# blachlylab/fade

Hardware: AMD Instinct MI355X
Metric: annotate reads/sec at 1/2/4/8 MI355X; rs/am tag bit-exact vs ref (higher is better)
Workload: dtype int16; 1 GPU; C2: 10000000 x 150 bp PE reads per GPU per step in 10 distinct batches, -w 100, --min-length 5, p_softclip 0.10; slots_in_flight=2, records_left_out=none

## Files before the change

fade_amd/csrc/fadehip.hip:

```cpp
#include "fadehip_kernels.hpp"
#include "bgzf_deflate.hpp"
#include "bgzf_inflate.hpp"
#include "bam_device.hpp"
#include "sw_stats.hpp"
#include <rccl/rccl.h>
#include <algorithm>
#include <chrono>
#include <condition_variable>
#include <cstdarg>
#include <cstdio>
#include <cstdlib>
#include <cstring>
#include <ctime>
#include <map>
#include <mutex>
#include <new>
#include <string>
#include <thread>
#include <unordered_map>
#include <vector>

using namespace fadehip;

namespace {
// ... 13 lines not shown
enum { A_TID, A_POS, A_LSEQ, A_CIGOFF, A_SEQOFF, A_FLAG, A_SA, A_CIG, A_SEQ, N_ARR };
struct Layout {
    size_t off[N_ARR], bytes[N_ARR], total;
};
Layout batch_layout(int64_t n, int64_t n_cig, int64_t n_seq) {
    Layout L;
    const size_t b[N_ARR] = {4 * (size_t)n, 4 * (size_t)n, 4 * (size_t)n, 4 * ((size_t)n + 1), 4 * ((size_t)n + 1),
                             2 * (size_t)n, (size_t)n,     4 * (size_t)n_cig, (size_t)n_seq};
    size_t at = 0;
    for (int k = 0; k < N_ARR; k++) {
        L.off[k] = at;
        L.bytes[k] = b[k];
        at += (b[k] + 8 + 255) & ~(size_t)255;
    }
    L.total = at;
    return L;
}

constexpr int64_t WIDE_MIN_SPAN = 1024;

struct Slot {
    hipStream_t stream = nullptr;
    hipStream_t score_stream = nullptr;
    DevBuf in[2];
    int cur = 0;
    bool have_batch = false;
    hipEvent_t ev_copied = nullptr;
    Layout L;
    PinBuf stage[2];
    const uint8_t *h_base = nullptr;
    struct Pending {
        bool valid = false;
        Layout L;
        const uint8_t *h_base = nullptr;
        uint32_t hist[NUM_LISTS] = {};
        int max_lq = 0;
        int l_seq_lo = 0, l_seq_hi = INT32_MAX;
        int64_t span_bound = 0;
        int n_reads = 0, n_skipped = 0;
        int buf = 0;
        uint32_t out_bound = 0;
        std::vector<std::pair<int64_t, int>> wide;
        } next;
    DevBuf rs, fwd, aln, trace;
    DevBuf ckpt, cand;
    DevBuf zblock;
    static constexpr size_t ZB_COUNTERS = 0, ZB_C64 = 128, ZB_SEL = 512, ZB_SEL_STRIDE = 48, ZB_STATS = 1024,
                            ZB_TICKETS = 1024 + 8 * 8 * STAT_PARTS, N_TICKETS = 256, ZB_PLAN = ZB_TICKETS + 4 * N_TICKETS,
                            ZB_BYTES = ZB_PLAN + 128;
    unsigned long long *d_counters64() const { return (unsigned long long *)((uint8_t *)zblock.p + ZB_C64); }
    unsigned long long *d_stats() const { return (unsigned long long *)((uint8_t *)zblock.p + ZB_STATS); }
    uint32_t *d_counters() const { return (uint32_t *)((uint8_t *)zblock.p + ZB_COUNTERS); }
    uint32_t *d_sel(int cls) const { return (uint32_t *)((uint8_t *)zblock.p + ZB_SEL + ZB_SEL_STRIDE * (size_t)cls); }
    uint32_t *d_ticket(int k) const { return (uint32_t *)((uint8_t *)zblock.p + ZB_TICKETS) + k; }
    PlanOut *d_plan() const { return (PlanOut *)((uint8_t *)zblock.p + ZB_PLAN); }
    bool sel_fresh[NUM_CLASSES] = {};
    int tickets_used = 0;
    DevBuf work[NUM_LISTS], meta[NUM_LISTS];
    DevBuf lrows;
    uint8_t *h_zb = nullptr;
    const uint32_t *h_counters() const { return (const uint32_t *)(h_zb + ZB_COUNTERS); }
    const unsigned long long *h_counters64() const { return (const unsigned long long *)(h_zb + ZB_C64); }
    const unsigned long long *h_stats() const { return (const unsigned long long *)(h_zb + ZB_STATS); }
    const PlanOut *h_plan() const { return (const PlanOut *)(h_zb + ZB_PLAN); }
    PinBuf res;
    size_t res_aln_off = 0;
    uint32_t bound[NUM_LISTS] = {};
    uint32_t hist[NUM_LISTS] = {};
    int64_t span_bound = 0;
    int max_lq = 0;
    int l_seq_lo = 0, l_seq_hi = INT32_MAX;
    uint32_t out_bound = 0, out_cap = 0;
    std::vector<std::pair<int64_t, int>> wide;
    bool use_ckpt = false;
    bool device_only = false;
    bool wide_all = false;
    int wave_lr_bound = 0, long_max_lq = 0, long_max_lr = 0;
    int floor_len = 0, window = 0;
// ... 46 lines not shown
    std::string err;
    std::mutex err_mu;
    Slot slots[FADEHIP_NUM_SLOTS];
    DevBuf genome, contig_len, contig_base;
    DevBuf l1_q, l1_r, l1_qn, l1_rn, l1_bad, l1_work, l1_aln;
    hipStream_t stats_stream = nullptr;
    DevBuf st_q, st_r, st_work, st_out, st_scratch;
    std::mutex stats_mu;
    BatchLane batch;
    int n_contigs = 0;
    std::vector<int64_t> h_contig_len;
    std::vector<uint64_t> h_contig_base;
    int cu_count = 0;
    hipStream_t copy_stream = nullptr;
    bool use_packed = true;
    bool two_pass = true;
    int tail_cus_per_xcd = 1;
    int score_g8 = 1;
    bool blocking_sync = false;
    int split_cus = 0;
    bool score_frame = true;
    bool score_persist = false;
    int p2_waves_fixed = 0;
    int span_slack = 24;
    bool debug = false;
    BgzfLane bgzf[FADEHIP_BGZF_LANES];
    InflateLane inf;
    bool bgzf_ready = false;
    int bgzf_geom_fixed = 0;
    double bgzf_last_ratio = 0;
    std::map<uint64_t, int> resident;
    std::mutex resident_mu;
};

namespace {

int set_err(fadehip_ctx *ctx, int code, const char *fmt, ...) {
    char buf[512];
    va_list ap;
    va_start(ap, fmt);
    vsnprintf(buf, sizeof buf, fmt, ap);
    va_end(ap);
    if (ctx) {
        std::lock_guard<std::mutex> l(ctx->err_mu);
        ctx->err = buf;
    }
// ... 331 lines not shown
    if (ctx->p2_waves_fixed > 0) p2_waves = std::min(ctx->p2_waves_fixed, bound_waves);
    p.p2_waves = (int)std::max<int64_t>(1, std::min<int64_t>(p2_waves, (c.budget / 2) / std::max<int64_t>((int64_t)p.wave_stride * 4, 1)));
    p.ckpt_bytes = (size_t)(p.chunk_oct * ck_bytes);
    p.fwd_bytes = (size_t)n_items * sizeof(Fwd);
    p.trace_bytes = (size_t)p.p2_waves * (size_t)p.wave_stride * 4;
    p.cand_bytes = sizeof(Cand) * (size_t)NUM_BUCKETS * (size_t)std::min<int64_t>(n_items, p.chunk_oct * 8);
    return 0;
}

int run_class_two_pass(fadehip_ctx *ctx, Slot &s, hipStream_t st, const ClassRun &c) {
    const int cls = c.cls, n_items = c.n_bound;
    TwoPassPlan p;
    int rc;
    if ((rc = plan_two_pass(ctx, s, c, p))) return rc;
    if ((rc = reserve_run(ctx, s.trash, s.ckpt, p.ckpt_bytes)) || (rc = reserve_run(ctx, s.trash, s.fwd, p.fwd_bytes)) ||
        (rc = reserve_run(ctx, s.trash, s.trace, p.trace_bytes)) || (rc = reserve_run(ctx, s.trash, s.cand, p.cand_bytes)))
        return rc;
    s.prof_counts[2] = std::max<int64_t>(s.prof_counts[2], (int64_t)p.trace_bytes);
    uint32_t *const sel_counters = s.d_sel(cls);
    const void *const score_fn = sw_kernel(cls, 1, p.longw), *const trace_fn = sw_kernel(cls, p.mode2, p.longw);
    if (!score_fn || !trace_fn) return set_err(ctx, FADEHIP_E_INVALID, "bad class %d", cls);
    bool framed = false;
    const void *const g8_fn = !p.longw && p.n_ck == 0 ? g8_kernel(ctx, cls, s.max_lq, 4 * p.n_blocks1, &framed) : nullptr;
    for (int64_t o0 = 0; o0 < p.total_oct; o0 += p.chunk_oct) {
        const int octs = (int)std::min<int64_t>(p.chunk_oct, p.total_oct - o0);
        const int i0 = (int)(o0 * 8);
        const int n = std::min(n_items - i0, octs * 8);
        if (!s.sel_fresh[cls]) HIPCHK(ctx, hipMemsetAsync(sel_counters, 0, sizeof(uint32_t) * NUM_BUCKETS, st));
        s.sel_fresh[cls] = false;
        SwArgs a = sw_args(ctx, s, c, i0, n);
        a.ref_stride = p.ref_stride1;
        a.ckpt = (uint32_t *)s.ckpt.p;
        a.ck_stride = p.ck_stride;
        a.n_ck = p.n_ck;
        a.count_dev = c.count_dev;
        a.item_base = (uint32_t)i0;
        a.sel.enabled = 1;
        a.sel.no_ckpt = p.n_ck == 0 ? 1 : 0;
        a.sel.meta = c.meta ? c.meta + i0 : nullptr;
        a.sel.floor_len = c.floor_len;
        a.sel.trace_all = ctx->prm.trace_all;
        a.sel.span_slack = ctx->span_slack;
        a.sel.cand = (Cand *)s.cand.p;
        a.sel.cap = (uint32_t)n;
        a.sel.bucket_n = sel_counters;
        a.sel.out = c.out;
// ... 7 lines not shown
            int ef = -1;
            if ((rc = record(ctx, s, &ef, st))) return rc;
            HIPCHK(ctx, hipStreamWaitEvent(sst, s.ev[ef], 0));
        }
        ChunkSpans sp{c.timed};
        if ((rc = sp.mark(ctx, s, 0, sst))) return rc;
        const void *fn1 = score_fn;
        int waves1 = octs;
        size_t lds = p.lds1;
        if (ctx->score_persist && class_rows(cls) == 10 && !p.longw && s.tickets_used < (int)Slot::N_TICKETS) {
            const int res = resident_waves(ctx, cls, 1, p.lds1, p.longw);
            const int cus = std::max(ctx->cu_count, 1), mine = s.score_stream ? std::max(cus - 8 * ctx->tail_cus_per_xcd, 1) : cus;
            fn1 = (const void *)sw_pk_kernel<10, 1, false, 16, true>;
            waves1 = std::max(1, std::min(octs, (int)((int64_t)res * mine / cus)));
            a.ticket = s.d_ticket(s.tickets_used++);
        } else if (g8_fn) {
            if (ctx->debug && o0 == 0) fprintf(stderr, "[fadehip] class of %d rows: score pass on eight-lane groups (longest read of the batch: %d), column-drift frame %s\n", 16 * class_rows(cls), s.max_lq, framed ? "on" : "off");
            fn1 = g8_fn;
            waves1 = (n + 15) / 16;
            lds = 2 * p.lds1;
        }
        if ((rc = launch_sw(ctx, fn1, waves1, lds, sst, a))) return rc;
        if ((rc = sp.mark(ctx, s, 1, sst))) return rc;
        if (sst != st) {
            int ej = sp.e[1];
            if (ej < 0 && (rc = record(ctx, s, &ej, sst))) return rc;
            HIPCHK(ctx, hipStreamWaitEvent(st, s.ev[ej], 0));
        }
        if (s.tickets_used >= (int)Slot::N_TICKETS)
            return set_err(ctx, FADEHIP_E_UNSUPPORTED, "more than %d pass-2 launches in one run (raise trace_bytes)", (int)Slot::N_TICKETS);
        SwArgs b2 = a;
        b2.sel.enabled = 0;
        b2.n_items = 0;
        b2.cand = (const Cand *)s.cand.p;
        b2.cand_cap = (uint32_t)n;
        b2.bucket_n = sel_counters;
        b2.cand_total = &s.d_plan()->cand_total;
        b2.trace = (uint32_t *)s.trace.p;
        b2.quad_stride = p.wave_stride;
        b2.count_dev = nullptr;
        b2.ticket = s.d_ticket(s.tickets_used++);
        b2.meta = c.meta ? c.meta + i0 : nullptr;
        b2.out = c.out;
        b2.rs = c.rs;
        b2.stats = (c.rs && c.gate) ? s.d_stats() : nullptr;
        b2.floor_len = c.floor_len;
        b2.gate = c.gate;
        b2.early_out = (c.gate && c.meta && !ctx->prm.trace_all) ? 1 : 0;
        b2.rerun_total = &s.d_plan()->rerun_total;
        if ((rc = launch_sw(ctx, trace_fn, std::min(p.p2_waves, octs + NUM_BUCKETS), p.lds1, st, b2))) return rc;
        if ((rc = sp.mark(ctx, s, 2, st))) return rc;
    }
    return 0;
}

int run_class_single(fadehip_ctx *ctx, Slot &s, hipStream_t st, const ClassRun &c) {
    const int cls = c.cls, R = class_rows(cls), n_items = c.n_bound, max_lr = c.max_lr;
    const bool packed = ctx->use_packed;
    const int per_wave = packed ? 8 : 4;
    const int n_blocks = (max_lr + 15 + 3) / 4;
    const uint64_t quad_stride = (uint64_t)n_blocks * (packed ? R : R / 2) * 64;
    const int ref_stride = packed ? std::min((((n_blocks * 4) * 2 + 15) / 16) * 16, (CH_COLS + 16) * 2) : (((n_blocks * 4) + 15) / 16) * 16;
    const size_t lds = (size_t)ref_stride * 4;
    if (lds > 64 * 1024)
        return set_err(ctx, FADEHIP_E_UNSUPPORTED, "reference window of %d bases needs %zu B LDS per wave (max 64 KiB)", max_lr, lds);
    const int64_t quad_bytes = (int64_t)quad_stride * 4;
    int64_t max_quads = std::max<int64_t>(1, c.budget / quad_bytes);
    const int total_quads = (n_items + per_wave - 1) / per_wave;
    const int64_t chunk_quads = std::min<int64_t>(max_quads, total_quads);
    int rc = reserve_run(ctx, s.trash, s.trace, (size_t)(chunk_quads * quad_bytes));
    if (rc) return rc;
    rc = reserve_run(ctx, s.trash, s.fwd, (size_t)n_items * sizeof(Fwd));
    if (rc) return rc;
    const void *const fn = sw_kernel(cls, packed ? 0 : SW_INT32, n_blocks > CH_BLOCKS);
// ... 130 lines not shown
    if (!s.stream) HIPCHK(ctx, hipStreamCreateWithFlags(&s.stream, hipStreamNonBlocking));
    HIPCHK(ctx, hipEventCreateWithFlags(&s.ev_copied, hipEventDisableTiming));
    HIPCHK(ctx, hipHostMalloc((void **)&s.h_zb, Slot::ZB_BYTES));
    memset(s.h_zb, 0, Slot::ZB_BYTES);
    if (ctx->tail_cus_per_xcd > 0 && ctx->cu_count >= 64 && ctx->cu_count % 32 == 0) {
        std::vector<uint32_t> mask((size_t)ctx->cu_count / 32, 0xffffffffu);
        for (int x = 0; x < 8 && 33 * x < ctx->cu_count; x++)
            for (int j = 0; j < ctx->tail_cus_per_xcd && j < 3; j++) {
                const int bit = 33 * x + 8 * j;
                if (bit < ctx->cu_count) mask[(size_t)bit / 32] &= ~(1u << (bit % 32));
            }
        if (const char *kv = getenv("FADEHIP_CU_MASK")) {
            size_t w = 0;
            for (const char *q = kv; *q && w < mask.size(); w++) {
                mask[w] = (uint32_t)strtoul(q, nullptr, 16);
                q = strchr(q, ',');
                if (!q) break;
                q++;
            }
        }
        if (hipExtStreamCreateWithCUMask(&s.score_stream, (uint32_t)mask.size(), mask.data()) != hipSuccess) {
            (void)hipGetLastError();
            s.score_stream = nullptr;
        }
    }
    return 0;
}

int check_slot(fadehip_ctx *ctx, int slot) {
    if (!ctx) return set_err(nullptr, FADEHIP_E_INVALID, "ctx is NULL");
    if (slot < 0 || slot >= FADEHIP_NUM_SLOTS) return set_err(ctx, FADEHIP_E_INVALID, "slot %d out of range", slot);
    return 0;
}

template <class T>
const T *d_arr(const Slot &s, int k) { return (const T *)((const uint8_t *)s.in[s.cur].p + s.L.off[k]); }

struct CigarSummary {
    int n_soft;
    uint32_t clipL, clipR;
    int64_t aligned;
};
inline CigarSummary summarize_cigar(const uint32_t *ops, uint32_t c0, uint32_t c1) {
    CigarSummary r = {0, 0, 0, 0};
    bool first = true;
    for (uint32_t k = c0; k < c1; k++) {
        const uint32_t op = ops[k] & 15u, len = ops[k] >> 4;
        if (op == 4) r.n_soft++;
// ... 53 lines not shown
    cr.floor_len = s.floor_len;
    cr.gate = 1;
    cr.budget = budget;
    cr.timed = true;
    return cr;
}

int enqueue_run(fadehip_ctx *ctx, Slot &s) {
    hipStream_t st = s.stream;
    const int n = s.n_reads;
    const int floor_len = s.floor_len;
    s.ev_used = 0;
    s.fwd_spans.clear();
    s.tb_spans.clear();
    s.tickets_used = 0;
    memset(s.prof_counts, 0, sizeof s.prof_counts);
    int rc;
    auto rsv = [&](DevBuf &b, size_t bytes) { return s.device_only ? reserve_roomy(ctx, b, bytes) : reserve(ctx, b, bytes); };
    uint32_t total_bound = 0;
    for (int c = 0; c < NUM_LISTS; c++) total_bound += s.bound[c];
    total_bound = std::min(total_bound, s.out_bound);
    s.out_cap = total_bound;
    s.res_aln_off = ((size_t)n + 255) & ~(size_t)255;
    if ((rc = rsv(s.rs, (size_t)n)) || (rc = rsv(s.aln, sizeof(fadehip_aln) * (size_t)std::max<uint32_t>(total_bound, 1))) ||
        (rc = reserve(ctx, s.zblock, Slot::ZB_BYTES)) ||
        (!s.device_only && (rc = reserve_pinned(ctx, s.res, s.res_aln_off + sizeof(fadehip_aln) * (size_t)total_bound))))
        return rc;
    for (int c = 0; c < NUM_LISTS; c++) {
        if (!s.bound[c]) continue;
        if ((rc = rsv(s.work[c], sizeof(Work) * (size_t)s.bound[c])) || (rc = rsv(s.meta[c], sizeof(Meta) * (size_t)s.bound[c])))
            return rc;
    }
    const int64_t budget = ctx->prm.trace_bytes > 0 ? ctx->prm.trace_bytes : ((int64_t)16 << 30);
    s.use_ckpt = s.last_cand * 32 > std::max<int64_t>(s.last_aln, 1);
    if (const char *kv = getenv("FADEHIP_CKPT")) s.use_ckpt = atoi(kv) != 0;
    if (ctx->two_pass) {
        size_t need_ckpt = 0, need_fwd = 0, need_trace = 0, need_cand = 0;
        for (int c = 0; c < NUM_CLASSES; c++) {
            if (!s.bound[c]) continue;
            TwoPassPlan p;
            if ((rc = plan_two_pass(ctx, s, level2_class_run(ctx, s, c, budget), p))) return rc;
            need_ckpt = std::max(need_ckpt, p.ckpt_bytes);
            need_fwd = std::max(need_fwd, p.fwd_bytes);
            need_trace = std::max(need_trace, p.trace_bytes);
            need_cand = std::max(need_cand, p.cand_bytes);
        }
        if ((rc = reserve_run(ctx, s.trash, s.ckpt, need_ckpt)) || (rc = reserve_run(ctx, s.trash, s.fwd, need_fwd)) ||
            (rc = reserve_run(ctx, s.trash, s.trace, need_trace)) || (rc = reserve_run(ctx, s.trash, s.cand, need_cand)))
            return rc;
    }
    HIPCHK(ctx, hipMemsetAsync(s.zblock.p, 0, Slot::ZB_BYTES, st));
    for (int c = 0; c < NUM_CLASSES; c++) s.sel_fresh[c] = true;
    if ((rc = record(ctx, s, &s.ev_gate0))) return rc;
    GateArgs g;
    memset(&g, 0, sizeof g);
    g.n_reads = n;
    g.tid = d_arr<int32_t>(s, A_TID);
    g.pos = d_arr<int32_t>(s, A_POS);
    g.l_seq = d_arr<int32_t>(s, A_LSEQ);
    g.flag = d_arr<uint16_t>(s, A_FLAG);
    g.has_sa = d_arr<uint8_t>(s, A_SA);
    g.cigar_off = d_arr<uint32_t>(s, A_CIGOFF);
    g.cigar_ops = d_arr<uint32_t>(s, A_CIG);
    g.seq_off = d_arr<uint32_t>(s, A_SEQOFF);
    g.floor_len = floor_len;
    g.window = s.window;
    g.n_contigs = ctx->n_contigs;
    g.contig_len = (const int64_t *)ctx->contig_len.p;
    g.contig_base = (const uint64_t *)ctx->contig_base.p;
    g.max_ref_len = ctx->prm.max_ref_len;
    g.wave_lr_bound = s.wave_lr_bound;
    g.long_lr_bound = s.long_max_lr;
    g.long_lq_bound = std::max(s.long_max_lq, 1);
    g.l_seq_lo = s.l_seq_lo;
    g.l_seq_hi = s.l_seq_hi;
    g.rs = (uint8_t *)s.rs.p;
    for (int c = 0; c < NUM_LISTS; c++) {
        g.work[c] = (Work *)s.work[c].p;
        g.meta[c] = (Meta *)s.meta[c].p;
        g.list_cap[c] = s.bound[c];
    }
    g.out_cap = s.out_cap;
    g.n_cigar_ops = (uint32_t)(s.L.bytes[A_CIG] / 4);
    g.n_seq_bytes = (uint32_t)s.L.bytes[A_SEQ];
    g.stats = s.d_stats();
    g.counters = s.d_counters();
    g.counters64 = s.d_counters64();
    hipLaunchKernelGGL(gate_kernel, dim3((n + GATE_BLOCK - 1) / GATE_BLOCK), dim3(GATE_BLOCK), 0, st, g);
    HIPCHK(ctx, hipGetLastError());
    if ((rc = record(ctx, s, &s.ev_gate1))) return rc;
    uint32_t exact[NUM_LISTS];
    for (int c = 0; c < NUM_LISTS; c++) exact[c] = s.bound[c];
    if (!ctx->two_pass) {
        HIPCHK(ctx, hipMemcpyAsync(s.h_zb, s.zblock.p, 128, hipMemcpyDeviceToHost, st));
        HIPCHK(ctx, hipStreamSynchronize(st));
        for (int c = 0; c < NUM_LISTS; c++) exact[c] = std::min(s.h_counters()[c], s.bound[c]);
    }
    for (int c = 0; c < NUM_CLASSES; c++) {
        if (!exact[c]) continue;
        ClassRun cr = level2_class_run(ctx, s, c, budget);
        cr.n_bound = (int)exact[c];
        rc = ctx->two_pass ? run_class_two_pass(ctx, s, st, cr) : run_class_single(ctx, s, st, cr);
        if (rc) return rc;
    }
    if (exact[LONG_LIST]) {
        ClassRun cr = level2_class_run(ctx, s, LONG_LIST, budget);
        cr.n_bound = (int)exact[LONG_LIST];
        if ((rc = run_long(ctx, s, st, cr, std::max(s.long_max_lq, 1)))) return rc;
    }
    if ((rc = record(ctx, s, &s.ev_end))) return rc;
    HIPCHK(ctx, hipMemcpyAsync(s.h_zb, s.zblock.p, Slot::ZB_BYTES, hipMemcpyDeviceToHost, st));
    if (s.device_only) return 0;
    HIPCHK(ctx, hipMemcpyAsync(s.res.p, s.rs.p, (size_t)n, hipMemcpyDeviceToHost, st));
    if (total_bound)
        HIPCHK(ctx, hipMemcpyAsync(s.res.p + s.res_aln_off, s.aln.p, sizeof(fadehip_aln) * (size_t)total_bound, hipMemcpyDeviceToHost, st));
    return 0;
}

int finish_run(fadehip_ctx *ctx, Slot &s, int slot) {
    if (s.state == 3) return 0;
    if (s.state != 2) return set_err(ctx, FADEHIP_E_STATE, "slot %d has not been run", slot);
    hipStream_t st = s.stream;
    const int n = s.n_reads;
    if (n == 0) {
        s.n_aln = 0;
        s.n_oversize = 0;
        memset(s.stats, 0, sizeof s.stats);
        s.stats[0] = s.n_skipped;
        s.state = 3;
        return 0;
    }
    HIPCHK(ctx, hipStreamSynchronize(st));
    for (void *q : s.trash) (void)hipFree(q);
    s.trash.clear();
    const uint32_t errbits = s.h_counters()[2 * NUM_LISTS];
    if (errbits) {
        s.state = 0;
        if (errbits & 64u) return set_err(ctx, FADEHIP_E_INVALID, "batch has a record whose cigar_off / seq_off are not non-decreasing within the arrays, or l_seq < 0");
        if (errbits & 8u) return set_err(ctx, FADEHIP_E_INVALID, "batch has a mapped soft-clipped record whose seq_packed slice is shorter than its l_seq");
        if (errbits & 16u) return set_err(ctx, FADEHIP_E_INVALID, "batch has a record whose cigar.alignedLength exceeds ref_span_bound=%lld", (long long)s.span_bound);
        if (errbits & 32u) return set_err(ctx, FADEHIP_E_INVALID, "batch has more records to re-align than its bounds said, or a read outside them (n_with_seq too small, or an l_seq outside l_seq_min / l_seq_max?)");
        return set_err(ctx, FADEHIP_E_INVALID, "batch has a mapped soft-clipped read whose tid is not a contig of the uploaded genome");
    }
    for (int c = 0; c < NUM_CLASSES; c++)
        if (s.bound[c]) {
            const uint32_t *bn = (const uint32_t *)(s.h_zb + Slot::ZB_SEL + Slot::ZB_SEL_STRIDE * (size_t)c);
            int octs = 0;
            for (int b = 0; b < NUM_BUCKETS; b++) octs += (int)((bn[b] + 7) / 8);
            s.p2_last_octs[c] = octs;
        }
    const uint32_t at = std::min(s.h_counters()[2 * NUM_LISTS + 3], s.out_cap);
    s.n_aln = (int)at;
    s.n_oversize = (int)s.h_counters()[2 * NUM_LISTS + 2];
    for (int k = 0; k < 8; k++) {
        s.stats[k] = 0;
        for (int q = 0; q < STAT_PARTS; q++) s.stats[k] += (int64_t)s.h_stats()[8 * q + k];
    }
    s.stats[0] += s.n_skipped;
    const PlanOut *po = s.h_plan();
    s.n_cand = (int64_t)po->cand_total;
    s.n_rerun = (int64_t)po->rerun_total;
    s.last_cand = s.n_cand;
    s.last_aln = (int64_t)at;
    s.prof_counts[0] = at;
    s.prof_counts[1] = (int64_t)s.h_counters64()[0 * C64_STRIDE];
// ... 236 lines not shown
    }
    if (strncmp(prop.gcnArchName, "gfx950", 6) != 0) {
        set_err(ctx, FADEHIP_E_NODEVICE, "device %d is %s; this library carries gfx950 code only", device, prop.gcnArchName);
        return fail(FADEHIP_E_NODEVICE);
    }
    ctx->cu_count = prop.multiProcessorCount;
    if (const char *kv = getenv("FADEHIP_KERNEL")) {
        ctx->use_packed = strcmp(kv, "int32") != 0;
        ctx->two_pass = strcmp(kv, "twopass") == 0;
    }
    if (ctx->prm.match > 2) ctx->two_pass = false;
    if (8 * (ctx->prm.match * FADEHIP_MAX_QUERY + ctx->prm.open + std::max(ctx->prm.match, 0)) >= 0x7c00) ctx->use_packed = false;
    if (!ctx->two_pass && ctx->prm.rules != FADEHIP_RULES_DEFAULT) {
        set_err(ctx, FADEHIP_E_UNSUPPORTED, "the rule switches exist on the two-pass path only (match <= 2, FADEHIP_KERNEL unset)");
        return fail(FADEHIP_E_UNSUPPORTED);
    }
    if (const char *kv = getenv("FADEHIP_SPAN_SLACK")) ctx->span_slack = atoi(kv);
    if (const char *kv = getenv("FADEHIP_TAIL_CUS")) ctx->tail_cus_per_xcd = std::max(0, std::min(atoi(kv), 8));
    if (const char *kv = getenv("FADEHIP_BAM_SPLIT")) ctx->split_cus = std::max(0, std::min(atoi(kv), 31));
    if (const char *kv = getenv("FADEHIP_P2_WAVES")) ctx->p2_waves_fixed = std::max(0, atoi(kv));
    if (const char *kv = getenv("FADEHIP_SCORE_PERSIST")) ctx->score_persist = atoi(kv) != 0;
    if (const char *kv = getenv("FADEHIP_SCORE_G8")) ctx->score_g8 = atoi(kv);
    if (const char *kv = getenv("FADEHIP_SCORE_FRAME")) ctx->score_frame = atoi(kv) != 0;
    ctx->debug = getenv("FADEHIP_DEBUG") != nullptr;
    uint8_t table[256];
    fill_ascii_table(table);
    if (hipStreamCreateWithFlags(&ctx->copy_stream, hipStreamNonBlocking) != hipSuccess ||
        hipMemcpyToSymbolAsync(HIP_SYMBOL(c_ascii_code), table, 256, 0, hipMemcpyHostToDevice, ctx->copy_stream) != hipSuccess ||
        hipStreamSynchronize(ctx->copy_stream) != hipSuccess) {
        set_err(ctx, FADEHIP_E_HIP, "hipMemcpyToSymbol failed: %s", hipGetErrorString(hipGetLastError()));
        return fail(FADEHIP_E_HIP);
    }
    static_assert(sizeof(uint32_t) * (2 * NUM_LISTS + 4) <= Slot::ZB_C64 - Slot::ZB_COUNTERS, "gate counters overflow their slice");
    static_assert(Slot::ZB_SEL + Slot::ZB_SEL_STRIDE * NUM_CLASSES <= Slot::ZB_STATS, "selection counters overlap the stats");
    static_assert(sizeof(uint32_t) * NUM_BUCKETS <= Slot::ZB_SEL_STRIDE, "selection counters overflow their slice");
    static_assert(sizeof(PlanOut) <= 128, "PlanOut overflows its slice");
    for (int k = 0; k < FADEHIP_NUM_SLOTS; k++)
        for (int c = 0; c < NUM_CLASSES; c++) ctx->slots[k].p2_last_octs[c] = -1;
    *out = ctx;
    return 0;
}

void fadehip_destroy(fadehip_ctx *ctx) {
    if (!ctx) return;
    (void)hipSetDevice(ctx->device);
    (void)hipDeviceSynchronize();
    for (int k = 0; k < FADEHIP_NUM_SLOTS; k++) {
        Slot &s = ctx->slots[k];
        for (DevBuf *b : {&s.in[0], &s.in[1], &s.rs, &s.fwd, &s.aln, &s.zblock, &s.trace, &s.ckpt, &s.cand, &s.lrows}) release(*b);
        for (void *q : s.trash) (void)hipFree(q);
        s.trash.clear();
        for (int c = 0; c < NUM_LISTS; c++) {
            release(s.work[c]);
            release(s.meta[c]);
        }
        release(s.stage[0]);
        release(s.stage[1]);
        release(s.res);
        if (s.ev_copied) (void)hipEventDestroy(s.ev_copied);
        for (hipEvent_t e : s.ev) (void)hipEventDestroy(e);
        if (s.h_zb) (void)hipHostFree(s.h_zb);
        if (s.score_stream) (void)hipStreamDestroy(s.score_stream);
        if (s.stream && s.stream != ctx->copy_stream) (void)hipStreamDestroy(s.stream);
    }
    if (ctx->copy_stream) (void)hipStreamDestroy(ctx->copy_stream);
    for (BgzfLane &l : ctx->bgzf) {
        for (DevBuf *b : {&l.src, &l.slots, &l.meta, &l.member_off}) release(*b);
        if (l.done) (void)hipEventDestroy(l.done);
        release(l.out);
        if (l.h_total) (void)hipHostFree(l.h_total);
        if (l.stream && (&l == &ctx->bgzf[0] || l.stream != ctx->bgzf[0].stream)) (void)hipStreamDestroy(l.stream);
    }
    for (DevBuf *b : {&ctx->inf.comp, &ctx->inf.blocks, &ctx->inf.out, &ctx->inf.status, &ctx->inf.ticket}) release(*b);
    release(ctx->inf.h_status);
    if (ctx->inf.stream) (void)hipStreamDestroy(ctx->inf.stream);
    release(ctx->genome);
    for (DevBuf *b : {&ctx->l1_q, &ctx->l1_r, &ctx->l1_qn, &ctx->l1_rn, &ctx->l1_bad, &ctx->l1_work, &ctx->l1_aln}) release(*b);
    for (DevBuf *b : {&ctx->st_q, &ctx->st_r, &ctx->st_work, &ctx->st_out, &ctx->st_scratch}) release(*b);
    if (ctx->stats_stream) (void)hipStreamDestroy(ctx->stats_stream);
    for (DevBuf *b : {&ctx->batch.in, &ctx->batch.meta, &ctx->batch.work, &ctx->batch.out}) release(*b);
    if (ctx->batch.stream) (void)hipStreamDestroy(ctx->batch.stream);
// ... 78 lines not shown
        if (lr > ctx->prm.max_ref_len)
            return set_err(ctx, FADEHIP_E_UNSUPPORTED, "reference %d has %lld bases (max_ref_len %d)", k, (long long)lr, ctx->prm.max_ref_len);
        Work w;
        w.r_base = (uint64_t)r_off[k];
        w.q_base = (uint32_t)q_off[k];
        w.lq = (uint32_t)lq;
        w.lr = (uint32_t)lr;
        w.idx = (uint32_t)k;
        w.flags = 0;
        w.out = 0;
        lists[cls].push_back(w);
        max_lr[cls] = std::max(max_lr[cls], (int)lr);
    }
    if (q_total >= (int64_t)1 << 32) return set_err(ctx, FADEHIP_E_UNSUPPORTED, "query bases per batch must stay below 2^32");
    DevBuf &d_q = ctx->l1_q, &d_r = ctx->l1_r, &d_qn = ctx->l1_qn, &d_rn = ctx->l1_rn, &d_bad = ctx->l1_bad,
           &d_work = ctx->l1_work, &d_aln = ctx->l1_aln;
    int rc = 0;
    hipStream_t st = s.stream;
    size_t n_work = 0;
    for (int c = 0; c < NUM_LISTS; c++) n_work += lists[c].size();
    if ((rc = reserve(ctx, d_q, (size_t)q_total + 2)) || (rc = reserve(ctx, d_r, (size_t)r_total + 2)) ||
        (rc = reserve(ctx, d_qn, (size_t)q_total / 2 + 8)) || (rc = reserve(ctx, d_rn, (size_t)r_total / 2 + 8)) ||
        (rc = reserve(ctx, d_bad, 4)) || (rc = reserve(ctx, d_aln, (size_t)n * sizeof(fadehip_aln))) ||
        (rc = reserve(ctx, d_work, std::max<size_t>(1, n_work) * sizeof(Work))) || (rc = reserve(ctx, s.zblock, Slot::ZB_BYTES)))
        return rc;
    HIPCHK(ctx, hipMemcpyAsync(d_q.p, q, (size_t)q_total, hipMemcpyHostToDevice, st));
    HIPCHK(ctx, hipMemcpyAsync(d_r.p, r, (size_t)r_total, hipMemcpyHostToDevice, st));
    HIPCHK(ctx, hipMemsetAsync(d_bad.p, 0, 4, st));
    if (q_total > 0)
        hipLaunchKernelGGL(pack_ascii_kernel, dim3((unsigned)((q_total / 2 + 256) / 256)), dim3(256), 0, st,
                           (const uint8_t *)d_q.p, (uint64_t)q_total, (uint64_t)0, (uint8_t *)d_qn.p, 0, (int *)d_bad.p);
    if (r_total > 0)
        hipLaunchKernelGGL(pack_ascii_kernel, dim3((unsigned)((r_total / 2 + 256) / 256)), dim3(256), 0, st,
                           (const uint8_t *)d_r.p, (uint64_t)r_total, (uint64_t)0, (uint8_t *)d_rn.p, 0, (int *)d_bad.p);
    HIPCHK(ctx, hipGetLastError());
    {
        size_t base = 0;
        for (int c = 0; c < NUM_LISTS; c++) {
            if (lists[c].empty()) continue;
            for (size_t k = 0; k < lists[c].size(); k++) lists[c][k].out = (uint32_t)(base + k);
            HIPCHK(ctx, hipMemcpyAsync((Work *)d_work.p + base, lists[c].data(), lists[c].size() * sizeof(Work), hipMemcpyHostToDevice, st));
            base += lists[c].size();
        }
    }
    const int64_t budget = ctx->prm.trace_bytes > 0 ? ctx->prm.trace_bytes : ((int64_t)4 << 30);
    {
        size_t base = 0;
        s.fwd_spans.clear();
        s.tb_spans.clear();
        s.tickets_used = 0;
        HIPCHK(ctx, hipMemsetAsync(s.zblock.p, 0, Slot::ZB_BYTES, st));
        for (int c = 0; c < NUM_CLASSES; c++) s.sel_fresh[c] = true;
        s.use_ckpt = true;
        if (const char *kv = getenv("FADEHIP_CKPT")) s.use_ckpt = atoi(kv) != 0;
        for (int c = 0; c < NUM_LISTS; c++) {
            if (lists[c].empty()) continue;
            hipLaunchKernelGGL(set_counts_kernel, dim3(1), dim3(1), 0, st, s.d_counters() + c, (uint32_t)lists[c].size());
            HIPCHK(ctx, hipGetLastError());
            ClassRun cr;
            cr.cls = c;
            cr.work = (const Work *)d_work.p + base;
            cr.n_bound = (int)lists[c].size();
            cr.count_dev = s.d_counters() + c;
            cr.max_lr = max_lr[c];
            cr.q_nib = (const uint8_t *)d_qn.p;
            cr.r_nib = (const uint8_t *)d_rn.p;
            cr.out = (fadehip_aln *)d_aln.p;
            cr.budget = budget;
            if (c == LONG_LIST) rc = run_long(ctx, s, st, cr, max_long_lq);
            else rc = ctx->two_pass ? run_class_two_pass(ctx, s, st, cr) : run_class_single(ctx, s, st, cr);
            if (rc) {
                (void)hipStreamSynchronize(st);
                return rc;
            }
            base += lists[c].size();
        }
        HIPCHK(ctx, hipStreamSynchronize(st));
// ... 393 lines not shown
        s.l_seq_lo = nx.l_seq_lo;
        s.l_seq_hi = nx.l_seq_hi;
        s.span_bound = nx.span_bound;
        s.out_bound = nx.out_bound;
        s.wide = nx.wide;
        s.n_reads = nx.n_reads;
        s.n_skipped = nx.n_skipped;
        s.have_batch = true;
        s.device_only = false;
        s.wide_all = false;
        s.next.valid = false;
        if (s.n_reads) HIPCHK(ctx, hipStreamWaitEvent(s.stream, s.ev_copied, 0));
    }
    s.floor_len = floor_len;
    s.window = window;
    if (s.n_reads == 0) {
        s.ev_gate0 = s.ev_gate1 = s.ev_end = -1;
        memset(s.prof_counts, 0, sizeof s.prof_counts);
        s.state = 2;
        return 0;
    }
    if ((rc = plan_run(ctx, s))) return rc;
    if ((rc = enqueue_run(ctx, s))) {
        (void)hipStreamSynchronize(s.stream);
        s.state = 0;
        return rc;
    }
    s.state = 2;
    return 0;
}

int fadehip_annotate_submit(fadehip_ctx *ctx, int slot, const fadehip_read_batch *batch, int32_t floor_len, int32_t window) {
    int rc = fadehip_annotate_upload(ctx, slot, batch);
    if (rc) return rc;
    return fadehip_annotate_run(ctx, slot, floor_len, window);
}

int fadehip_annotate_results(fadehip_ctx *ctx, int slot, fadehip_anno_view *out) {
    int rc = check_slot(ctx, slot);
    if (rc) return rc;
    if (!out) return set_err(ctx, FADEHIP_E_INVALID, "out is NULL");
    Slot &s = ctx->slots[slot];
    HIPCHK(ctx, hipSetDevice(ctx->device));
    if ((rc = finish_run(ctx, s, slot))) return rc;
    out->rs = s.n_reads ? s.res.p : nullptr;
    out->aln = s.n_aln ? (const fadehip_aln *)(s.res.p + s.res_aln_off) : nullptr;
// ... 1179 lines not shown
```

fade_amd/csrc/fadehip_kernels.hpp:

```cpp
#pragma once
#include <type_traits>
#include <hip/hip_runtime.h>
#include <stdint.h>
#include "../../include/fadehip.h"

namespace fadehip {

__host__ __device__ constexpr uint64_t make_class_lut() {
    uint64_t v = 0;
    for (int k = 0; k < 16; k++) {
        uint64_t c = 5;
        if (k == 1) c = 0;
        if (k == 2) c = 1;
        if (k == 4) c = 2;
        if (k == 8) c = 3;
        if (k == 15) c = 4;
        v |= c << (4 * k);
    }
    return v;
}
__host__ __device__ constexpr uint64_t make_comp_lut() {
    const int t[16] = {0, 8, 4, 12, 2, 10, 6, 14, 1, 9, 5, 13, 3, 11, 7, 15};
    uint64_t v = 0;
    for (int k = 0; k < 16; k++) v |= (uint64_t)t[k] << (4 * k);
// ... 1833 lines not shown
    }
}

__device__ __forceinline__ uint32_t traceback_one(const TbArgs &a, const int item) {
    int n_items = a.n_items;
    if (a.count_dev) n_items = min(n_items, max(0, (int)*a.count_dev - (int)a.item_base));
    if (item >= n_items) return 0u;
    if (a.packed == 3)
        return traceback_path(a, item, 0, a.trace + (uint64_t)item * a.quad_stride, 0, 0, item);
    const uint64_t trace_off = (uint64_t)(a.packed ? (item >> 3) : (item >> 2)) * a.quad_stride;
    return traceback_path(a, item, 0, a.trace + trace_off, a.packed ? ((item >> 1) & 3) : (item & 3), item & 1, item);
}

__global__ void traceback_kernel(TbArgs a) {
    const uint32_t r = traceback_one(a, (int)(blockIdx.x * blockDim.x + threadIdx.x));
    if (a.stats) add_artifact_stats(a.stats, r, blockIdx.x);
}

struct PlanOut {
    unsigned long long cand_total;
    unsigned long long rerun_total;
};

__global__ void set_counts_kernel(uint32_t *dst, uint32_t v) { *dst = v; }

}
```

Measured before the change: 1.239 billion reads/s.

## Copy alignments to host after score pass and patch pass-2 results via gather list

When a run has a single two-pass class, the alignment array is copied to the host right after the score pass, overlapping the D2H transfer with pass 2. Pass 2 runs on a separate tail stream, which can be CU-masked to the CUs the score stream leaves free. A new gather kernel then collects the pass-2 entries into a compact patch list that is applied on the host. The zero-block is also double-buffered, so the next run's memset is issued at the end of the current run instead of at its start. This adds a host patch loop and a fallback full copy if the candidate list overflows, along with more cross-stream event dependencies.

```diff
diff --git a/fade_amd/csrc/fadehip.hip b/fade_amd/csrc/fadehip.hip
--- a/fade_amd/csrc/fadehip.hip
+++ b/fade_amd/csrc/fadehip.hip
@@ -59,6 +59,13 @@
 struct Slot {
     hipStream_t stream = nullptr;
     hipStream_t score_stream = nullptr;
+    std::vector<uint32_t> score_mask;
+    hipStream_t tail_stream = nullptr;
+    bool tail_tried = false;
+    bool early = false;
+    DevBuf patch;
+    PinBuf h_patch;
+    uint32_t patch_cap = 0, patch_sent = 0;
     DevBuf in[2];
     int cur = 0;
     bool have_batch = false;
@@ -82,15 +89,18 @@
     DevBuf rs, fwd, aln, trace;
     DevBuf ckpt, cand;
     DevBuf zblock;
+    size_t zoff = 0;
+    bool zb_next_clean = false;
     static constexpr size_t ZB_COUNTERS = 0, ZB_C64 = 128, ZB_SEL = 512, ZB_SEL_STRIDE = 48, ZB_STATS = 1024,
                             ZB_TICKETS = 1024 + 8 * 8 * STAT_PARTS, N_TICKETS = 256, ZB_PLAN = ZB_TICKETS + 4 * N_TICKETS,
-                            ZB_BYTES = ZB_PLAN + 128;
-    unsigned long long *d_counters64() const { return (unsigned long long *)((uint8_t *)zblock.p + ZB_C64); }
-    unsigned long long *d_stats() const { return (unsigned long long *)((uint8_t *)zblock.p + ZB_STATS); }
-    uint32_t *d_counters() const { return (uint32_t *)((uint8_t *)zblock.p + ZB_COUNTERS); }
-    uint32_t *d_sel(int cls) const { return (uint32_t *)((uint8_t *)zblock.p + ZB_SEL + ZB_SEL_STRIDE * (size_t)cls); }
-    uint32_t *d_ticket(int k) const { return (uint32_t *)((uint8_t *)zblock.p + ZB_TICKETS) + k; }
-    PlanOut *d_plan() const { return (PlanOut *)((uint8_t *)zblock.p + ZB_PLAN); }
+                            ZB_BYTES = ZB_PLAN + 128, ZB_STRIDE = (ZB_BYTES + 255) & ~(size_t)255;
+    uint8_t *zb() const { return (uint8_t *)zblock.p + zoff; }
+    unsigned long long *d_counters64() const { return (unsigned long long *)(zb() + ZB_C64); }
+    unsigned long long *d_stats() const { return (unsigned long long *)(zb() + ZB_STATS); }
+    uint32_t *d_counters() const { return (uint32_t *)(zb() + ZB_COUNTERS); }
+    uint32_t *d_sel(int cls) const { return (uint32_t *)(zb() + ZB_SEL + ZB_SEL_STRIDE * (size_t)cls); }
+    uint32_t *d_ticket(int k) const { return (uint32_t *)(zb() + ZB_TICKETS) + k; }
+    PlanOut *d_plan() const { return (PlanOut *)(zb() + ZB_PLAN); }
     bool sel_fresh[NUM_CLASSES] = {};
     int tickets_used = 0;
     DevBuf work[NUM_LISTS], meta[NUM_LISTS];
@@ -183,6 +193,9 @@
     bool score_frame = true;
     bool score_persist = false;
     int p2_waves_fixed = 0;
+    bool early_copy = true;
+    int early_tail = 0;
+    int patch_cap = 4096;
     int span_slack = 24;
     bool debug = false;
     BgzfLane bgzf[FADEHIP_BGZF_LANES];
@@ -560,6 +573,8 @@
     if (!score_fn || !trace_fn) return set_err(ctx, FADEHIP_E_INVALID, "bad class %d", cls);
     bool framed = false;
     const void *const g8_fn = !p.longw && p.n_ck == 0 ? g8_kernel(ctx, cls, s.max_lq, 4 * p.n_blocks1, &framed) : nullptr;
+    if (p.total_oct > p.chunk_oct) s.early = false;
+    const bool early = s.early;
     for (int64_t o0 = 0; o0 < p.total_oct; o0 += p.chunk_oct) {
         const int octs = (int)std::min<int64_t>(p.chunk_oct, p.total_oct - o0);
         const int i0 = (int)(o0 * 8);
@@ -613,10 +628,19 @@
         }
         if ((rc = launch_sw(ctx, fn1, waves1, lds, sst, a))) return rc;
         if ((rc = sp.mark(ctx, s, 1, sst))) return rc;
-        if (sst != st) {
+        hipStream_t p2st = st;
+        if (sst != st || early) {
             int ej = sp.e[1];
             if (ej < 0 && (rc = record(ctx, s, &ej, sst))) return rc;
-            HIPCHK(ctx, hipStreamWaitEvent(st, s.ev[ej], 0));
+            if (sst != st) HIPCHK(ctx, hipStreamWaitEvent(st, s.ev[ej], 0));
+            if (early) {
+                if (s.tail_stream) {
+                    p2st = s.tail_stream;
+                    HIPCHK(ctx, hipStreamWaitEvent(p2st, s.ev[ej], 0));
+                }
+                HIPCHK(ctx, hipMemcpyAsync(s.res.p + s.res_aln_off, s.aln.p, sizeof(fadehip_aln) * (size_t)s.out_cap, hipMemcpyDeviceToHost,
+                                           s.tail_stream ? st : sst));
+            }
         }
         if (s.tickets_used >= (int)Slot::N_TICKETS)
             return set_err(ctx, FADEHIP_E_UNSUPPORTED, "more than %d pass-2 launches in one run (raise trace_bytes)", (int)Slot::N_TICKETS);
@@ -639,8 +663,26 @@
         b2.gate = c.gate;
         b2.early_out = (c.gate && c.meta && !ctx->prm.trace_all) ? 1 : 0;
         b2.rerun_total = &s.d_plan()->rerun_total;
-        if ((rc = launch_sw(ctx, trace_fn, std::min(p.p2_waves, octs + NUM_BUCKETS), p.lds1, st, b2))) return rc;
-        if ((rc = sp.mark(ctx, s, 2, st))) return rc;
+        if ((rc = launch_sw(ctx, trace_fn, std::min(p.p2_waves, octs + NUM_BUCKETS), p.lds1, p2st, b2))) return rc;
+        if ((rc = sp.mark(ctx, s, 2, p2st))) return rc;
+        if (early) {
+            PatchArgs pa;
+            pa.cand = b2.cand;
+            pa.cand_cap = b2.cand_cap;
+            pa.bucket_n = sel_counters;
+            pa.work = b2.work;
+            pa.out = c.out;
+            pa.out_cap = s.out_cap;
+            pa.head = (PatchHead *)s.patch.p;
+            pa.list = (PatchEntry *)((uint8_t *)s.patch.p + sizeof(PatchHead));
+            pa.cap = s.patch_cap;
+            const uint32_t blocks = std::max<uint32_t>(1, std::min<uint32_t>(64, (s.patch_sent * (uint32_t)(sizeof(PatchEntry) / 4) + 255) / 256));
+            hipLaunchKernelGGL(patch_gather_kernel, dim3(blocks), dim3(256), 0, p2st, pa);
+            HIPCHK(ctx, hipGetLastError());
+            int et = -1;
+            if ((rc = record(ctx, s, &et, s.tail_stream ? p2st : sst))) return rc;
+            HIPCHK(ctx, hipStreamWaitEvent(st, s.ev[et], 0));
+        }
     }
     return 0;
 }
@@ -817,8 +859,26 @@
         if (hipExtStreamCreateWithCUMask(&s.score_stream, (uint32_t)mask.size(), mask.data()) != hipSuccess) {
             (void)hipGetLastError();
             s.score_stream = nullptr;
-        }
-    }
+        } else {
+            s.score_mask = mask;
+        }
+    }
+    return 0;
+}
+
+int ensure_tail(fadehip_ctx *ctx, Slot &s) {
+    if (s.tail_stream || s.tail_tried) return 0;
+    s.tail_tried = true;
+    if (ctx->early_tail == 1 && !s.score_mask.empty()) {
+        std::vector<uint32_t> mask(s.score_mask.size());
+        uint32_t any = 0;
+        for (size_t w = 0; w < mask.size(); w++) any |= (mask[w] = ~s.score_mask[w]);
+        if (any && hipExtStreamCreateWithCUMask(&s.tail_stream, (uint32_t)mask.size(), mask.data()) != hipSuccess) {
+            (void)hipGetLastError();
+            s.tail_stream = nullptr;
+        }
+    }
+    if (!s.tail_stream) HIPCHK(ctx, hipStreamCreateWithFlags(&s.tail_stream, hipStreamNonBlocking));
     return 0;
 }
 
@@ -918,8 +978,9 @@
     total_bound = std::min(total_bound, s.out_bound);
     s.out_cap = total_bound;
     s.res_aln_off = ((size_t)n + 255) & ~(size_t)255;
+    if (s.zblock.cap < 2 * Slot::ZB_STRIDE) s.zb_next_clean = false, s.zoff = 0;
     if ((rc = rsv(s.rs, (size_t)n)) || (rc = rsv(s.aln, sizeof(fadehip_aln) * (size_t)std::max<uint32_t>(total_bound, 1))) ||
-        (rc = reserve(ctx, s.zblock, Slot::ZB_BYTES)) ||
+        (rc = reserve(ctx, s.zblock, 2 * Slot::ZB_STRIDE)) ||
         (!s.device_only && (rc = reserve_pinned(ctx, s.res, s.res_aln_off + sizeof(fadehip_aln) * (size_t)total_bound))))
         return rc;
     for (int c = 0; c < NUM_LISTS; c++) {
@@ -945,7 +1006,35 @@
             (rc = reserve_run(ctx, s.trash, s.trace, need_trace)) || (rc = reserve_run(ctx, s.trash, s.cand, need_cand)))
             return rc;
     }
-    HIPCHK(ctx, hipMemsetAsync(s.zblock.p, 0, Slot::ZB_BYTES, st));
+    {
+        int n_cls = 0;
+        for (int c = 0; c < NUM_CLASSES; c++) n_cls += s.bound[c] ? 1 : 0;
+        const char *why = nullptr;
+        if (!ctx->early_copy) why = "FADEHIP_EARLY_COPY=0";
+        else if (!ctx->two_pass) why = "single-pass kernels";
+        else if (s.device_only) why = "results stay on the device";
+        else if (n_cls != 1) why = "not exactly one class list";
+        else if (s.bound[LONG_LIST]) why = "long list";
+        else if (ctx->prm.trace_all) why = "trace_all";
+        else if (s.last_cand * 2 > ctx->patch_cap) why = "the previous run's candidates exceed half the patch list";
+        else if (s.use_ckpt) why = "snapshots";
+        else if (!total_bound) why = "no alignments";
+        s.early = why == nullptr;
+        if (s.early) {
+            s.patch_cap = (uint32_t)ctx->patch_cap;
+            s.patch_sent = (uint32_t)std::min<int64_t>(s.patch_cap, 2 * s.last_cand + 64);
+            const size_t bytes = sizeof(PatchHead) + sizeof(PatchEntry) * (size_t)std::max<uint32_t>(s.patch_cap, 1);
+            if (((ctx->early_tail || !s.score_stream) && (rc = ensure_tail(ctx, s))) || (rc = reserve(ctx, s.patch, bytes)) ||
+                (rc = reserve_pinned(ctx, s.h_patch, bytes)))
+                return rc;
+        }
+        if (ctx->debug)
+            fprintf(stderr, "[fadehip] copy order: %s (%s)\n", s.early ? "early" : "late",
+                    !s.early ? why : !s.tail_stream ? "the copy on the score stream" : ctx->early_tail == 1 && !s.score_mask.empty() ? "pass 2 on the CUs the score mask leaves free" : "pass 2 on a plain stream");
+    }
+    if (s.zb_next_clean) s.zoff ^= Slot::ZB_STRIDE;
+    else HIPCHK(ctx, hipMemsetAsync(s.zb(), 0, Slot::ZB_BYTES, st));
+    s.zb_next_clean = false;
     for (int c = 0; c < NUM_CLASSES; c++) s.sel_fresh[c] = true;
     if ((rc = record(ctx, s, &s.ev_gate0))) return rc;
     GateArgs g;
@@ -988,7 +1077,7 @@
     uint32_t exact[NUM_LISTS];
     for (int c = 0; c < NUM_LISTS; c++) exact[c] = s.bound[c];
     if (!ctx->two_pass) {
-        HIPCHK(ctx, hipMemcpyAsync(s.h_zb, s.zblock.p, 128, hipMemcpyDeviceToHost, st));
+        HIPCHK(ctx, hipMemcpyAsync(s.h_zb, s.zb(), 128, hipMemcpyDeviceToHost, st));
         HIPCHK(ctx, hipStreamSynchronize(st));
         for (int c = 0; c < NUM_LISTS; c++) exact[c] = std::min(s.h_counters()[c], s.bound[c]);
     }
@@ -1005,10 +1094,14 @@
         if ((rc = run_long(ctx, s, st, cr, std::max(s.long_max_lq, 1)))) return rc;
     }
     if ((rc = record(ctx, s, &s.ev_end))) return rc;
-    HIPCHK(ctx, hipMemcpyAsync(s.h_zb, s.zblock.p, Slot::ZB_BYTES, hipMemcpyDeviceToHost, st));
+    HIPCHK(ctx, hipMemcpyAsync(s.h_zb, s.zb(), Slot::ZB_BYTES, hipMemcpyDeviceToHost, st));
+    HIPCHK(ctx, hipMemsetAsync((uint8_t *)s.zblock.p + (s.zoff ^ Slot::ZB_STRIDE), 0, Slot::ZB_BYTES, st));
+    s.zb_next_clean = true;
     if (s.device_only) return 0;
     HIPCHK(ctx, hipMemcpyAsync(s.res.p, s.rs.p, (size_t)n, hipMemcpyDeviceToHost, st));
-    if (total_bound)
+    if (s.early)
+        HIPCHK(ctx, hipMemcpyAsync(s.h_patch.p, s.patch.p, sizeof(PatchHead) + sizeof(PatchEntry) * (size_t)s.patch_sent, hipMemcpyDeviceToHost, st));
+    else if (total_bound)
         HIPCHK(ctx, hipMemcpyAsync(s.res.p + s.res_aln_off, s.aln.p, sizeof(fadehip_aln) * (size_t)total_bound, hipMemcpyDeviceToHost, st));
     return 0;
 }
@@ -1037,6 +1130,27 @@
         if (errbits & 16u) return set_err(ctx, FADEHIP_E_INVALID, "batch has a record whose cigar.alignedLength exceeds ref_span_bound=%lld", (long long)s.span_bound);
         if (errbits & 32u) return set_err(ctx, FADEHIP_E_INVALID, "batch has more records to re-align than its bounds said, or a read outside them (n_with_seq too small, or an l_seq outside l_seq_min / l_seq_max?)");
         return set_err(ctx, FADEHIP_E_INVALID, "batch has a mapped soft-clipped read whose tid is not a contig of the uploaded genome");
+    }
+    if (s.early) {
+        s.early = false;
+        const PatchHead head = *(const PatchHead *)s.h_patch.p;
+        const PatchEntry *const list = (const PatchEntry *)(s.h_patch.p + sizeof(PatchHead));
+        uint8_t *const h_aln = s.res.p + s.res_aln_off;
+        if (head.overflow || head.n > s.patch_cap) {
+            HIPCHK(ctx, hipMemcpyAsync(h_aln, s.aln.p, sizeof(fadehip_aln) * (size_t)s.out_cap, hipMemcpyDeviceToHost, st));
+            HIPCHK(ctx, hipStreamSynchronize(st));
+        } else {
+            if (head.n > s.patch_sent) {
+                HIPCHK(ctx, hipMemcpyAsync((void *)(list + s.patch_sent), (const uint8_t *)s.patch.p + sizeof(PatchHead) + sizeof(PatchEntry) * (size_t)s.patch_sent,
+                                           sizeof(PatchEntry) * (size_t)(head.n - s.patch_sent), hipMemcpyDeviceToHost, st));
+                HIPCHK(ctx, hipStreamSynchronize(st));
+            }
+            for (uint32_t k = 0; k < head.n; k++)
+                if (list[k].out < s.out_cap) memcpy(h_aln + sizeof(fadehip_aln) * (size_t)list[k].out, &list[k].e, sizeof(fadehip_aln));
+        }
+        if (ctx->debug)
+            fprintf(stderr, "[fadehip] slot %d: patch list of %u entries (%u sent with the run)%s\n", slot, head.n, s.patch_sent,
+                    head.overflow ? ", overflow: the array was copied again" : "");
     }
     for (int c = 0; c < NUM_CLASSES; c++)
         if (s.bound[c]) {
@@ -1319,6 +1433,9 @@
     if (const char *kv = getenv("FADEHIP_SCORE_PERSIST")) ctx->score_persist = atoi(kv) != 0;
     if (const char *kv = getenv("FADEHIP_SCORE_G8")) ctx->score_g8 = atoi(kv);
     if (const char *kv = getenv("FADEHIP_SCORE_FRAME")) ctx->score_frame = atoi(kv) != 0;
+    if (const char *kv = getenv("FADEHIP_EARLY_COPY")) ctx->early_copy = atoi(kv) != 0;
+    if (const char *kv = getenv("FADEHIP_EARLY_TAIL")) ctx->early_tail = strcmp(kv, "masked") == 0 ? 1 : strcmp(kv, "plain") == 0 ? 2 : 0;
+    if (const char *kv = getenv("FADEHIP_PATCH_CAP")) ctx->patch_cap = std::max(0, std::min(atoi(kv), 1 << 20));
     ctx->debug = getenv("FADEHIP_DEBUG") != nullptr;
     uint8_t table[256];
     fill_ascii_table(table);
@@ -1354,6 +1471,9 @@
         release(s.stage[0]);
         release(s.stage[1]);
         release(s.res);
+        release(s.patch);
+        release(s.h_patch);
+        if (s.tail_stream) (void)hipStreamDestroy(s.tail_stream);
         if (s.ev_copied) (void)hipEventDestroy(s.ev_copied);
         for (hipEvent_t e : s.ev) (void)hipEventDestroy(e);
         if (s.h_zb) (void)hipHostFree(s.h_zb);
@@ -1478,7 +1598,7 @@
     if ((rc = reserve(ctx, d_q, (size_t)q_total + 2)) || (rc = reserve(ctx, d_r, (size_t)r_total + 2)) ||
         (rc = reserve(ctx, d_qn, (size_t)q_total / 2 + 8)) || (rc = reserve(ctx, d_rn, (size_t)r_total / 2 + 8)) ||
         (rc = reserve(ctx, d_bad, 4)) || (rc = reserve(ctx, d_aln, (size_t)n * sizeof(fadehip_aln))) ||
-        (rc = reserve(ctx, d_work, std::max<size_t>(1, n_work) * sizeof(Work))) || (rc = reserve(ctx, s.zblock, Slot::ZB_BYTES)))
+        (rc = reserve(ctx, d_work, std::max<size_t>(1, n_work) * sizeof(Work))) || (rc = reserve(ctx, s.zblock, 2 * Slot::ZB_STRIDE)))
         return rc;
     HIPCHK(ctx, hipMemcpyAsync(d_q.p, q, (size_t)q_total, hipMemcpyHostToDevice, st));
     HIPCHK(ctx, hipMemcpyAsync(d_r.p, r, (size_t)r_total, hipMemcpyHostToDevice, st));
@@ -1505,10 +1625,13 @@
         s.fwd_spans.clear();
         s.tb_spans.clear();
         s.tickets_used = 0;
-        HIPCHK(ctx, hipMemsetAsync(s.zblock.p, 0, Slot::ZB_BYTES, st));
+        s.zoff = 0;
+        s.zb_next_clean = false;
+        HIPCHK(ctx, hipMemsetAsync(s.zb(), 0, Slot::ZB_BYTES, st));
         for (int c = 0; c < NUM_CLASSES; c++) s.sel_fresh[c] = true;
         s.use_ckpt = true;
         if (const char *kv = getenv("FADEHIP_CKPT")) s.use_ckpt = atoi(kv) != 0;
+        s.early = false;
         for (int c = 0; c < NUM_LISTS; c++) {
             if (lists[c].empty()) continue;
             hipLaunchKernelGGL(set_counts_kernel, dim3(1), dim3(1), 0, st, s.d_counters() + c, (uint32_t)lists[c].size());
@@ -1948,6 +2071,8 @@
     }
     if ((rc = plan_run(ctx, s))) return rc;
     if ((rc = enqueue_run(ctx, s))) {
+        if (s.tail_stream) (void)hipStreamSynchronize(s.tail_stream);
+        if (s.score_stream) (void)hipStreamSynchronize(s.score_stream);
         (void)hipStreamSynchronize(s.stream);
         s.state = 0;
         return rc;
diff --git a/fade_amd/csrc/fadehip_kernels.hpp b/fade_amd/csrc/fadehip_kernels.hpp
--- a/fade_amd/csrc/fadehip_kernels.hpp
+++ b/fade_amd/csrc/fadehip_kernels.hpp
@@ -1879,6 +1879,56 @@
     unsigned long long rerun_total;
 };
 
+struct PatchHead {
+    uint32_t n;
+    uint32_t overflow;
+    uint32_t pad[2];
+};
+struct PatchEntry {
+    uint32_t out;
+    uint32_t pad;
+    fadehip_aln e;
+};
+static_assert(sizeof(fadehip_aln) % 4 == 0 && sizeof(PatchEntry) == 8 + sizeof(fadehip_aln), "the gather copies dwords");
+struct PatchArgs {
+    const Cand *cand;
+    uint32_t cand_cap;
+    const uint32_t *bucket_n;
+    const Work *work;
+    const fadehip_aln *out;
+    uint32_t out_cap;
+    PatchHead *head;
+    PatchEntry *list;
+    uint32_t cap;
+};
+
+__global__ __launch_bounds__(256) void patch_gather_kernel(PatchArgs a) {
+    constexpr uint32_t ENTRY_DW = sizeof(PatchEntry) / 4;
+    uint32_t first[NUM_BUCKETS + 1];
+    first[0] = 0;
+#pragma unroll
+    for (int b = 0; b < NUM_BUCKETS; b++) first[b + 1] = first[b] + min(a.bucket_n[b], a.cand_cap);
+    const uint32_t total = first[NUM_BUCKETS], live = min(total, a.cap);
+    if (blockIdx.x == 0 && threadIdx.x == 0) {
+        a.head->n = total;
+        a.head->overflow = total > a.cap ? 1u : 0u;
+        a.head->pad[0] = a.head->pad[1] = 0;
+    }
+    uint32_t *const dst = (uint32_t *)a.list;
+    for (uint64_t at = (uint64_t)blockIdx.x * blockDim.x + threadIdx.x; at < (uint64_t)live * ENTRY_DW; at += (uint64_t)gridDim.x * blockDim.x) {
+        const uint32_t p = (uint32_t)(at / ENTRY_DW), d = (uint32_t)(at % ENTRY_DW);
+        int b = 0;
+#pragma unroll
+        for (int k = 1; k < NUM_BUCKETS; k++) b += p >= first[k] ? 1 : 0;
+        const Cand c = a.cand[(uint64_t)b * a.cand_cap + (p - first[b])];
+        const uint32_t o = a.work[c.src].out;
+        uint32_t v;
+        if (o >= a.out_cap) v = d == 0 ? 0xffffffffu : 0u;
+        else v = d == 0 ? o : d == 1 ? 0u : ((const uint32_t *)(a.out + o))[d - 2];
+        dst[at] = v;
+    }
+}
+
 __global__ void set_counts_kernel(uint32_t *dst, uint32_t v) { *dst = v; }
 
 }
```

Measured after the change: 1.297 billion reads/s (median of 6 runs). 4.7% higher.
